# MarkJhonBao/InfantPoseEstimation_GaussianBias

Measured on AMD Instinct MI355X. Metric: images/sec (train fwd+bwd) HRFormer-S 256x192, higher is better.
Workload: dtype bf16; 1 GPU; HRFormer-small + fusion head, 256x192 -> 64x48, K=17, train step fwd+bwd+AdamW, DropPath 0.1, BN train; global_batch=64, per_gpu_batch=64, parallelism=dp1, launch=hipGraph replay, branches on concurrent HIP streams

## Files before the change

include/posekernels.h:

```cpp
#ifndef POSEKERNELS_H
#define POSEKERNELS_H

#include <stdint.h>

#ifdef __cplusplus
extern "C" {
#endif

#define PK_OK 0
#define PK_ERR_INVALID (-1)
#define PK_ERR_UNSUPPORTED (-2)

#define PK_DT_F32 0
#define PK_DT_BF16 1

int pk_version(void);
const char* pk_last_error_string(void);
int pk_marker(int id, void* stream);

int pk_gaussian_target(const float* keypoints, const float* visible, const float* lut, int lut_len,
                       float* target, float* weight, int B, int K, int Hh, int Wh,
                       double stride_x, double stride_y, double reach, int patch_n, int patch_c, void* stream);

int pk_dense_target(const float* keypoints, const float* visible, float* heatmaps, float* weights,
// ... 51 lines not shown
                       int B, int K, int H, int W, float sigma_t, const float* lambdas7, void* stream);

int pk_fusion_terms_fwd(const float* heatmaps, const float* offsets, const float* variances, const float* target,
                        const float* weight, const float* gt_keypoints, const float* coords, float* ws, float* losses, float* sigma,
                        int B, int K, int H, int W, float in_w, float in_h, float sigma_t,
                        const float* lambdas7, int use_target_weight, void* stream);
int pk_fusion_terms_bwd(const float* heatmaps, const float* target, const float* ws, const float* grad_total,
                        const float* grad_sigma, const float* grad_losses ,
                        float* d_heatmaps, float* d_offsets, float* d_variances, float* d_coords,
                        int B, int K, int H, int W, float sigma_t, const float* lambdas7, void* stream);
int pk_local_gaussian_refine(const float* heatmaps, const float* coords_in, float* coords_out, int BK, int H, int W,
                             int local_radius, void* stream);
int pk_softargmax_bwd(const float* heatmaps, const float* coords, const float* scores, const float* grad_coords,
                      const float* grad_scores, float* d_heatmaps, int BK, int H, int W, void* stream);

#define PK_REDUCE_BLOCKS 1024
int pk_pixel_loss_fwd(const float* pred, const float* target, const float* weight, float* partial, float* loss,
                      int B, int K, int HW, int kind, void* stream);
int pk_pixel_loss_bwd(const float* pred, const float* target, const float* weight, const float* grad_out,
                      float* d_pred, int B, int K, int HW, int kind, void* stream);
int pk_spatial_stats(const float* heatmaps, float* mean, float* var, int BK, int H, int W, void* stream);
int pk_spatial_stats_bwd(const float* heatmaps, const float* mean, const float* var, const float* grad_mean, const float* grad_var,
                         float* grad_heatmaps, int BK, int H, int W, void* stream);

int pk_adamw_step(float* param, const float* grad, float* exp_avg, float* exp_avg_sq, const uint8_t* decay_mask,
                  uint16_t* param_bf16, int64_t n, const float* lr_dev, const int32_t* step_dev,
                  float beta1, float beta2, float eps, float weight_decay, float grad_scale, void* stream);



int pk_conv2d_nhwc(const void* x, const void* w_packed, void* out, float* stats_partial, const float* bias,
                   int B, int Hs, int Ws, int Cin, int Cout, int ksize, int stride, int dilated_input, int Ho, int Wo,
                   int act, int out_mode, const void* addend, void* stream);
int pk_conv2d_affine_nhwc(const void* x, const void* w_packed, void* out, const float* col_scale, const float* col_shift,
                          const void* residual, int relu, int B, int Hs, int Ws, int Cin, int Cout, int ksize, int stride, int Ho,
                          int Wo, void* stream);
int pk_conv_stats_tiles(int M);
#define PK_GROUP_MAX 12
typedef struct PkConvDesc {
    const void* x; const void* w; void* out;
    float* stats;
    const float* col_scale;
    const float* bias;
    const void* res;
    int B, Hs, Ws, Cin, Cout, ksize, stride, dilated_input, Ho, Wo;
    int act;
} PkConvDesc;
int pk_conv2d_group(const PkConvDesc* descs, int n, void* stream);
typedef struct PkBnFwdDesc {
    const void* raw; const float* stats_partial; const float* gamma; const float* beta;
    float* running_mean; float* running_var; int64_t* num_batches_tracked;
    const void* residual; void* y; float* save_mean; float* save_rstd; uint8_t* relu_mask ;
    int64_t rows; int tiles, C; float momentum, eps; int relu;
} PkBnFwdDesc;
int pk_bn_train_fwd_group(const PkBnFwdDesc* descs, int n, void* stream);
typedef struct PkBnBwdDesc {
    const void* dy; const void* y_act; const void* raw; const float* save_mean; const float* save_rstd; const float* gamma;
    float* partial; float* dgamma; float* dbeta; void* dx; void* dresidual; const uint8_t* relu_mask ;
    int64_t rows; int C; int relu;
} PkBnBwdDesc;
int pk_bn_bwd_group_blocks(int64_t rows);
int pk_bn_bwd_group(const PkBnBwdDesc* descs, int n, void* stream);
typedef struct PkFuseDesc {
    const void* inputs[4]; int in_h[4]; int in_w[4]; int n_inputs;
    void* out; const void* mask_y; int B, H, W, C, relu;
} PkFuseDesc;
// ... 114 lines not shown
```

infantposeestimation_gaussianbias_amd/csrc/pk_igemm.hip:

```cpp
#include "pk_common.h"

typedef __attribute__((ext_vector_type(8))) short bf16x8;
typedef __attribute__((ext_vector_type(4))) float f32x4;

#define STAT_ROWS 128
#define BKK 32
#define LDS_PITCH 40

struct IgemmArgs {
    const uint16_t* x;
    const uint16_t* w;
    void* out;
    const float* bias;
    const float* col_scale;
    const uint16_t* res;
    const float* res_scale;
    const int32_t* a_rowmap;
    const int32_t* o_rowmap;
    float* stats;
    uint16_t* preact;
    const uint16_t* gelu_of;
    int M, N, Cin, T;
    int Hs, Ws;
    int Ho, Wo;
// ... 562 lines not shown
template <int BM, int BN, int WM, int WN, int BK, int LEAN>
__global__ void __launch_bounds__(256) __attribute__((amdgpu_waves_per_eu(2))) k_igemm2(IgemmArgs p_in) {
    igemm2_body<BM, BN, WM, WN, BK, LEAN>(p_in, (int)blockIdx.x, (int)blockIdx.y, (int)gridDim.x, (int)gridDim.y);
}

struct IgemmGroup {
    IgemmArgs a[PK_GROUP_MAX];
    int first[PK_GROUP_MAX + 1];
    int gy[PK_GROUP_MAX];
    int n;
};
template <int BM, int BN, int WM, int WN, int BK, int LEAN>
__global__ void __launch_bounds__(256) __attribute__((amdgpu_waves_per_eu(2))) k_igemm2g(IgemmGroup g) {
    const int L = (int)blockIdx.x;
    int i = 0;
    while (i + 1 < g.n && L >= g.first[i + 1]) ++i;
    const int local = L - g.first[i], gy = g.gy[i], gx = (g.first[i + 1] - g.first[i]) / gy;
    igemm2_body<BM, BN, WM, WN, BK, LEAN>(g.a[i], local % gx, local / gx, gx, gy);
}

#define C8_STAGE 32768
#define C8_STAGES 5
template <int OFF>
__device__ __forceinline__ bf16x8 c8_read(uint32_t lds_byte_addr) {
    bf16x8 v;
    asm volatile("ds_read_b128 %0, %1 offset:%2" : "=v"(v) : "v"(lds_byte_addr), "n"(OFF) : "memory");
    return v;
}
__device__ __forceinline__ void c8_fence4(bf16x8& a, bf16x8& b, bf16x8& c, bf16x8& d) {
    asm volatile("s_waitcnt lgkmcnt(0)" : "+v"(a), "+v"(b), "+v"(c), "+v"(d)::"memory");
}
__device__ __forceinline__ void c8_barrier() { asm volatile("s_barrier" ::: "memory"); }

__global__ void __launch_bounds__(512, 2) k_conv8p(IgemmArgs p) {
    __shared__ __attribute__((aligned(1024))) uint16_t c8_smem[C8_STAGES * C8_STAGE / 2];
    const int tid = threadIdx.x, lane = tid & 63;
    const int wave = __builtin_amdgcn_readfirstlane(tid >> 6);
    const int grp = wave >> 2;
    const int wn = wave & 3;
    int mt, nt;
    {
        const int G = gridDim.x, L = blockIdx.x, q = G >> 3, r = G & 7, xcd = L & 7;
        const int tile = (xcd < r ? xcd * (q + 1) : r * (q + 1) + (xcd - r) * q) + (L >> 3);
        const int ntiles = p.N >> 8;
        mt = tile / ntiles;
        nt = tile - mt * ntiles;
    }
    const int m0 = mt * 256, n0 = nt * 256;
    const auto rx = __builtin_amdgcn_make_buffer_rsrc(const_cast<uint16_t*>(p.x), 0, 0x7ffffff0, 0x00020000);
    const auto rw = __builtin_amdgcn_make_buffer_rsrc(const_cast<uint16_t*>(p.w), 0, 0x7ffffff0, 0x00020000);
    const uint32_t lds0 = (uint32_t)(uintptr_t)(__attribute__((address_space(3))) void*)c8_smem;

    const int drow = wave * 16 + (lane >> 2);
    const int lchunk = (lane & 3) ^ (((lane >> 5) & 1) << 1);
    unsigned pc[2];
    int pedge[2];
    unsigned wo[2];
    {
        const int hw = p.Ho * p.Wo;
#pragma unroll
        for (int i = 0; i < 2; ++i) {
            const int m = m0 + i * 128 + drow;
            pc[i] = OOB_OFF;
            pedge[i] = 0;
            if (m < p.M) {
                const int b = m / hw, rr = m - b * hw, oy = rr / p.Wo, ox = rr - oy * p.Wo;
                pc[i] = (unsigned)(((b * p.Hs + oy) * p.Ws + ox) * p.Cin + lchunk * 8) * 2u;
                pedge[i] = (oy > 0 ? 1 : 0) | (oy < p.Hs - 1 ? 2 : 0) | (ox > 0 ? 4 : 0) | (ox < p.Ws - 1 ? 8 : 0);
            }
            wo[i] = (unsigned)(((n0 + i * 128 + drow) * p.T) * p.Cin + lchunk * 8) * 2u;
        }
    }
    const int nk = p.T * (p.Cin >> 5);
    int q_tap = 0, q_c0 = 0, q_need = 0, q_delta = 0;
    auto set_tap = [&]() {
        if (p.T == 9) {
            const int kh = q_tap / 3, kw = q_tap - kh * 3;
            q_need = (kh == 0 ? 1 : 0) | (kh == 2 ? 2 : 0) | (kw == 0 ? 4 : 0) | (kw == 2 ? 8 : 0);
            q_delta = ((kh - 1) * p.Ws + (kw - 1)) * p.Cin * 2;
        }
    };
    set_tap();
    auto issue_tile = [&](int stage) {
#if defined(__HIP_DEVICE_COMPILE__)
        uint16_t* sp = c8_smem + (stage * C8_STAGE + wave * 1024) / 2;
#pragma unroll
        for (int i = 0; i < 2; ++i) {
            const bool ok = pc[i] != OOB_OFF && (pedge[i] & q_need) == q_need;
            __builtin_amdgcn_raw_ptr_buffer_load_lds(rx, (__attribute__((address_space(3))) void*)(sp + i * 4096), 16,
                                                     ok ? pc[i] + (unsigned)q_delta : OOB_OFF, q_c0 * 2, 0, 0);
        }
#pragma unroll
        for (int i = 0; i < 2; ++i)
            __builtin_amdgcn_raw_ptr_buffer_load_lds(rw, (__attribute__((address_space(3))) void*)(sp + 8192 + i * 4096), 16, wo[i],
                                                     (q_tap * p.Cin + q_c0) * 2, 0, 0);
#endif
        if (++q_tap == p.T) {
            q_tap = 0;
            q_c0 += 32;
        }
        set_tap();
    };

    const int frow = lane & 15;
    const uint32_t fchunk = (uint32_t)(((lane >> 4) ^ ((frow >> 3) << 1)) * 16);
    const uint32_t faddr_p = lds0 + (grp * 128 + frow) * 64 + fchunk;
    const uint32_t faddr_w = lds0 + 16384 + (wn * 64 + frow) * 64 + fchunk;

    f32x4 acc[4][8];
#pragma unroll
    for (int a = 0; a < 4; ++a)
#pragma unroll
        for (int b = 0; b < 8; ++b) acc[a][b] = (f32x4){0.f, 0.f, 0.f, 0.f};

    issue_tile(0);
    issue_tile(1);
    issue_tile(2);
    asm volatile("s_waitcnt vmcnt(8)" ::: "memory");
    c8_barrier();
    int st_r = 0, st_w = 3;
    bf16x8 wf[4], pf[8];
    auto multiply = [&]() {
        c8_fence4(wf[0], wf[1], wf[2], wf[3]);
        c8_fence4(pf[0], pf[1], pf[2], pf[3]);
        c8_fence4(pf[4], pf[5], pf[6], pf[7]);
        __builtin_amdgcn_sched_barrier(0);
        __builtin_amdgcn_s_setprio(1);
#pragma unroll
        for (int b = 0; b < 8; ++b)
#pragma unroll
            for (int a = 0; a < 4; ++a) acc[a][b] = __builtin_amdgcn_mfma_f32_16x16x32_bf16(wf[a], pf[b], acc[a][b], 0, 0, 0);
        __builtin_amdgcn_s_setprio(0);
// ... 1 lines not shown
    };
    for (int t = 0; t <= nk; ++t) {
        if (grp == 1 && t > 0) multiply();
        if (t < nk) {
            const uint32_t bp = faddr_p + st_r * C8_STAGE, bw = faddr_w + st_r * C8_STAGE;
            wf[0] = c8_read<0>(bw);
            wf[1] = c8_read<1024>(bw);
            wf[2] = c8_read<2048>(bw);
            wf[3] = c8_read<3072>(bw);
            pf[0] = c8_read<0>(bp);
            pf[1] = c8_read<1024>(bp);
            pf[2] = c8_read<2048>(bp);
            pf[3] = c8_read<3072>(bp);
            pf[4] = c8_read<4096>(bp);
            pf[5] = c8_read<5120>(bp);
            pf[6] = c8_read<6144>(bp);
            pf[7] = c8_read<7168>(bp);
            if (t + 3 < nk) issue_tile(st_w);
            __builtin_amdgcn_sched_barrier(0);
            if (grp == 0) multiply();
        }
        if (t + 3 < nk) {
            asm volatile("s_waitcnt vmcnt(8)" ::: "memory");
        } else if (t + 2 < nk) {
            asm volatile("s_waitcnt vmcnt(4)" ::: "memory");
        } else {
            asm volatile("s_waitcnt vmcnt(0)" ::: "memory");
        }
        st_r = st_r == C8_STAGES - 1 ? 0 : st_r + 1;
        st_w = st_w == C8_STAGES - 1 ? 0 : st_w + 1;
        c8_barrier();
    }

    if (p.stats && m0 + grp * 128 < p.M) {
        float* dst = p.stats + (size_t)(mt * 2 + grp) * 2 * p.N + n0 + wn * 64;
#pragma unroll
        for (int a = 0; a < 4; ++a)
#pragma unroll
            for (int r = 0; r < 4; ++r) {
                float sm = 0.f, sq = 0.f;
#pragma unroll
                for (int b = 0; b < 8; ++b) {
                    const float v = acc[a][b][r];
                    sm += v;
                    sq += v * v;
                }
                sm = row16_sum(sm);
                sq = row16_sum(sq);
                if ((lane & 15) == 0) {
                    const int nl = a * 16 + (lane >> 4) * 4 + r;
                    dst[nl] = sm;
                    dst[p.N + nl] = sq;
                }
            }
    }
    uint16_t* stage = c8_smem + wave * 8192;
    if (p.col_scale) {
#pragma unroll
        for (int a = 0; a < 4; ++a) {
            const int c = n0 + wn * 64 + a * 16 + (lane >> 4) * 4;
            const f32x4 sc = *reinterpret_cast<const f32x4*>(p.col_scale + c), sh = *reinterpret_cast<const f32x4*>(p.bias + c);
#pragma unroll
            for (int b = 0; b < 8; ++b) {
                acc[a][b] = acc[a][b] * sc + sh;
                if (p.act == 3) {
#pragma unroll
                    for (int r = 0; r < 4; ++r) acc[a][b][r] = fmaxf(acc[a][b][r], 0.f);
                }
            }
        }
    }
#pragma unroll
    for (int a = 0; a < 4; ++a)
#pragma unroll
        for (int b = 0; b < 8; ++b) {
            const int px = b * 16 + (lane & 15);
            const int chunk = (a * 2 + (lane >> 5)) ^ (px & 7);
            uint2 v;
            v.x = pack_bf16x2(acc[a][b][0], acc[a][b][1]);
            v.y = pack_bf16x2(acc[a][b][2], acc[a][b][3]);
            *reinterpret_cast<uint2*>(stage + px * 64 + chunk * 8 + ((lane >> 4) & 1) * 4) = v;
        }
    __builtin_amdgcn_fence(__ATOMIC_ACQ_REL, "wavefront");
    __builtin_amdgcn_wave_barrier();
    uint16_t* out = reinterpret_cast<uint16_t*>(p.out);
#pragma unroll 4
    for (int it = 0; it < 16; ++it) {
        const int px = it * 8 + (lane >> 3), ch = lane & 7;
        const int m = m0 + grp * 128 + px;
        const u32x4 v = *reinterpret_cast<const u32x4*>(stage + px * 64 + ((ch ^ (px & 7)) * 8));
        if (m < p.M) *reinterpret_cast<u32x4*>(out + (size_t)m * p.ldo + n0 + wn * 64 + ch * 8) = v;
    }
}
typedef __attribute__((ext_vector_type(2))) unsigned int u32x2;
template <int OFF>
__device__ __forceinline__ bf16x8 h3_read(uint32_t lds_byte_addr) {
    bf16x8 v;
    asm volatile("ds_read_b128 %0, %1 offset:%2" : "=v"(v) : "v"(lds_byte_addr), "n"(OFF) : "memory");
    return v;
}
__device__ __forceinline__ int h3_div(int q, int d, float inv) {
    int r = (int)((float)q * inv);
    const int rem = q - r * d;
    r += rem >= d ? 1 : (rem < 0 ? -1 : 0);
    return r;
}
__device__ __forceinline__ void h3_wait_vm(int n) {
#define H3_W(k) case k: asm volatile("s_waitcnt vmcnt(" #k ")" ::: "memory"); break;
    switch (n < 0 ? 0 : (n > 63 ? 63 : n)) {
        H3_W(0) H3_W(1) H3_W(2) H3_W(3) H3_W(4) H3_W(5) H3_W(6) H3_W(7) H3_W(8) H3_W(9) H3_W(10) H3_W(11) H3_W(12) H3_W(13) H3_W(14) H3_W(15)
        H3_W(16) H3_W(17) H3_W(18) H3_W(19) H3_W(20) H3_W(21) H3_W(22) H3_W(23) H3_W(24) H3_W(25) H3_W(26) H3_W(27) H3_W(28) H3_W(29) H3_W(30) H3_W(31)
        H3_W(32) H3_W(33) H3_W(34) H3_W(35) H3_W(36) H3_W(37) H3_W(38) H3_W(39) H3_W(40) H3_W(41) H3_W(42) H3_W(43) H3_W(44) H3_W(45) H3_W(46) H3_W(47)
        H3_W(48) H3_W(49) H3_W(50) H3_W(51) H3_W(52) H3_W(53) H3_W(54) H3_W(55) H3_W(56) H3_W(57) H3_W(58) H3_W(59) H3_W(60) H3_W(61) H3_W(62) H3_W(63)
    }
#undef H3_W
}
template <int CIN, int COUT>
__global__ void __launch_bounds__(256, 2) k_conv3h(IgemmArgs p, int pieces_per_wave) {
    constexpr int RB = CIN * 2, CH = CIN / 8, RP = 1024 / RB, KS = CIN / 32, NI = COUT / 32;
    extern __shared__ __attribute__((aligned(1024))) uint16_t h3_smem[];
    const int tid = threadIdx.x, lane = tid & 63;
    const int wave = __builtin_amdgcn_readfirstlane(tid >> 6);
    const int wm = wave >> 1, wn = wave & 1;
    const int H = p.Hs, W = p.Ws, W2 = W + 2, P = (H + 2) * W2, halo = W + 3;
    const int nsamples = p.M / (H * W), Mp = nsamples * P;
    const int ntiles = (Mp + 127) >> 7;
// ... 317 lines not shown
    }
    PK_REQUIRE((int64_t)M * (ldo > Cin ? ldo : Cin) < 0x3fffffffLL, "%s: tensor too large for 32-bit byte offsets", who);
    return PK_OK;
}

extern "C" int pk_conv2d_nhwc(const void* x, const void* w_packed, void* out, float* stats_partial, const float* bias,
                              int B, int Hs, int Ws, int Cin, int Cout, int ksize, int stride, int dilated_input, int Ho,
                              int Wo, int act, int out_mode, const void* addend, void* stream) {
    const int M = B * Ho * Wo;
    int rc = check_common("pk_conv2d_nhwc", x, w_packed, out, M, Cout, Cin, Cout, out_mode);
    if (rc) return rc;
    PK_REQUIRE(ksize == 1 || ksize == 3, "pk_conv2d_nhwc: ksize %d", ksize);
    PK_REQUIRE(stride == 1 || (stride == 2 && !dilated_input), "pk_conv2d_nhwc: stride %d", stride);
    PK_REQUIRE(B > 0 && Hs > 0 && Ws > 0 && Ho > 0 && Wo > 0, "pk_conv2d_nhwc: bad geometry");
    if (dilated_input) {
        PK_REQUIRE(Ho <= 2 * Hs && Wo <= 2 * Ws && Ho >= 2 * Hs - 1 && Wo >= 2 * Ws - 1, "pk_conv2d_nhwc: dilated geometry %dx%d <- %dx%d", Ho, Wo, Hs, Ws);
    } else {
        const int pad = ksize / 2;
        PK_REQUIRE(Ho == (Hs + 2 * pad - ksize) / stride + 1 && Wo == (Ws + 2 * pad - ksize) / stride + 1,
                   "pk_conv2d_nhwc: output %dx%d does not match input %dx%d k=%d s=%d", Ho, Wo, Hs, Ws, ksize, stride);
    }
    PK_REQUIRE(out_mode >= 0 && out_mode <= 2 && act >= 0 && act <= 2, "pk_conv2d_nhwc: bad mode");
    PK_REQUIRE((int64_t)B * Hs * Ws * Cin < 0x3fffffffLL && (int64_t)Cout * ksize * ksize * Cin < 0x3fffffffLL,
               "pk_conv2d_nhwc: input too large for 32-bit byte offsets");
    PK_REQUIRE(out_mode == 2 || (Cout & 3) == 0, "pk_conv2d_nhwc: Cout=%d must be a multiple of 4 for row-major output", Cout);
    IgemmArgs a{};
    a.x = (const uint16_t*)x; a.w = (const uint16_t*)w_packed; a.out = out; a.bias = bias; a.stats = stats_partial;
    a.M = M; a.N = Cout; a.Cin = Cin; a.T = ksize * ksize; a.Hs = Hs; a.Ws = Ws; a.Ho = Ho; a.Wo = Wo;
    a.stride = stride; a.pad = ksize / 2; a.dilated = dilated_input; a.ldo = Cout; a.rows_per_sample = Ho * Wo;
    a.act = act; a.out_mode = out_mode;
    PK_REQUIRE(!addend || (out_mode == 0 && !stats_partial), "pk_conv2d_nhwc: an addend needs the bf16 row-major output and no statistics");
    a.res = (const uint16_t*)addend;
    return igemm_launch(a, (hipStream_t)stream, "pk_conv2d_nhwc");
}

extern "C" int pk_conv2d_affine_nhwc(const void* x, const void* w_packed, void* out, const float* col_scale, const float* col_shift,
                                     const void* residual, int relu, int B, int Hs, int Ws, int Cin, int Cout, int ksize, int stride, int Ho,
                                     int Wo, void* stream) {
    const int M = B * Ho * Wo;
    int rc = check_common("pk_conv2d_affine_nhwc", x, w_packed, out, M, Cout, Cin, Cout, 0);
    if (rc) return rc;
    PK_REQUIRE(col_scale && col_shift, "pk_conv2d_affine_nhwc: null scale / shift");
    PK_REQUIRE((ksize == 1 || ksize == 3) && (stride == 1 || stride == 2), "pk_conv2d_affine_nhwc: ksize %d stride %d", ksize, stride);
    PK_REQUIRE(B > 0 && Hs > 0 && Ws > 0 && Ho > 0 && Wo > 0, "pk_conv2d_affine_nhwc: bad geometry");
    const int pad = ksize / 2;
    PK_REQUIRE(Ho == (Hs + 2 * pad - ksize) / stride + 1 && Wo == (Ws + 2 * pad - ksize) / stride + 1,
               "pk_conv2d_affine_nhwc: output %dx%d does not match input %dx%d k=%d s=%d", Ho, Wo, Hs, Ws, ksize, stride);
    PK_REQUIRE((int64_t)B * Hs * Ws * Cin < 0x3fffffffLL && (int64_t)Cout * ksize * ksize * Cin < 0x3fffffffLL,
               "pk_conv2d_affine_nhwc: input too large for 32-bit byte offsets");
    PK_REQUIRE((Cout & 3) == 0, "pk_conv2d_affine_nhwc: Cout=%d must be a multiple of 4", Cout);
    IgemmArgs a{};
    a.x = (const uint16_t*)x; a.w = (const uint16_t*)w_packed; a.out = out; a.bias = col_shift; a.col_scale = col_scale;
    a.M = M; a.N = Cout; a.Cin = Cin; a.T = ksize * ksize; a.Hs = Hs; a.Ws = Ws; a.Ho = Ho; a.Wo = Wo;
    a.stride = stride; a.pad = pad; a.dilated = 0; a.ldo = Cout; a.rows_per_sample = Ho * Wo;
    a.act = relu ? 3 : 0; a.out_mode = 0; a.res = (const uint16_t*)residual;
    return igemm_launch(a, (hipStream_t)stream, "pk_conv2d_affine_nhwc");
}

extern "C" int pk_conv2d_group(const PkConvDesc* d, int n, void* stream) {
    PK_REQUIRE(d && n > 0 && n <= PK_GROUP_MAX, "pk_conv2d_group: 1..%d members, got %d", PK_GROUP_MAX, n);
    IgemmGroup g{};
    bool k64 = true;
    int total = 0;
    for (int i = 0; i < n; ++i) {
        const PkConvDesc& c = d[i];
        const int M = c.B * c.Ho * c.Wo;
// ... 1209 lines not shown
```

infantposeestimation_gaussianbias_amd/dispatch.py:

```python
import contextlib
import os

import torch

from . import nnops
from ._lib import PoseKernelError

_ACTIVE = []


def backend_for(model):
    ok = getattr(model, "_pk_supported", None)
    if ok is None:
        ok = nnops.supported(model)
        object.__setattr__(model, "_pk_supported", ok)
    if not ok:
        raise PoseKernelError(
            f"{type(model).__name__}: layer shapes outside the HIP kernels (channels must be multiples of 8, head_dim a multiple of 8 "
            "up to 64, window 7) and no 8-aligned padded twin could be built (models/padded.py); there is no fallback path")
    return nnops


def padded_twin(model):
    if getattr(model, "_pk_twin", None) is False:
        return None
    from .models import padded
    return padded.twin_for(model)


def backend_name(model) -> str:
    if torch.cuda.is_available() and padded_twin(model) is not None:
        return "hip (8-aligned padded twin)"
    backend_for(model)
    return "hip"


@contextlib.contextmanager
def scope(model):
    if _ACTIVE:
        yield _ACTIVE[-1]
        return
    ops = backend_for(model)
    _ACTIVE.append(ops)
    try:
        with nnops.use_weights(model):
            yield ops
            join_detached()
    finally:
        _ACTIVE.pop()


def ops():
    if not _ACTIVE:
        raise RuntimeError("network op called outside dispatch.scope(model)")
    return _ACTIVE[-1]


from .nnops import (backward_milestone, conv_bn_act, deconv_bn_relu, drop_scales, exchange, exchange_output, head_out, mlp_rows, residual_block,
                    to_features, window_attention_tokens, window_block)


def to_public(x):
    ops()
    return x.permute(0, 3, 1, 2)


def from_public(x):
    ops()
    if x.dtype != nnops.ACT_DTYPE:
        B, C, H, W = x.shape
        if x.requires_grad and torch.is_grad_enabled() and C % 8 == 0:
            return x.permute(0, 2, 3, 1).to(nnops.ACT_DTYPE).contiguous()
        return nnops.to_features(x, cpad=-(-C // 8) * 8)
    return x.permute(0, 2, 3, 1).contiguous()


_SIDE = {}
_STREAMS_OFF = [False]
_REGION = [False]
_EVENTS = []


def set_streams(enabled: bool):
    _STREAMS_OFF[0] = not enabled


def set_region_mode(enabled: bool):
    _REGION[0] = bool(enabled)


def streams_enabled() -> bool:
# ... 179 lines not shown
```

infantposeestimation_gaussianbias_amd/models/fusion_head.py:

```python
import math
from typing import Dict, Optional, Tuple

import torch
import torch.nn as nn

from .. import hipops
from .. import dispatch as nnops
from ._blocks import conv


class SoftArgmax2D(nn.Module):

    def __init__(self, beta: float = 1.0):
        super().__init__()
        self.beta = beta

    def forward(self, heatmaps: torch.Tensor) -> Tuple[torch.Tensor, torch.Tensor]:
        h = heatmaps.float()
        if torch.is_grad_enabled() and h.requires_grad:
            co, sc = hipops.softargmax(h)
            if self.beta != 1.0:
                co = hipops.softargmax(h * self.beta)[0]
            return co, sc
        one = torch.full((1,), 40.0, device=heatmaps.device)
# ... 31 lines not shown
    seq = nn.ModuleDict({"0": conv(cin, hidden, 3), "1": nn.BatchNorm2d(hidden), "3": nn.Conv2d(hidden, cout, 1)})
    return seq


class HeatmapRegressionHead(nn.Module):
    def __init__(self, in_channels: int, num_keypoints: int = 17, hidden_dim: int = 256, use_subpixel_refinement: bool = True):
        super().__init__()
        self.in_channels, self.num_keypoints, self.use_subpixel_refinement = in_channels, num_keypoints, use_subpixel_refinement
        self.shared_layers = nn.ModuleDict({"0": conv(in_channels, hidden_dim, 3), "1": nn.BatchNorm2d(hidden_dim),
                                            "3": conv(hidden_dim, hidden_dim, 3), "4": nn.BatchNorm2d(hidden_dim)})
        self.heatmap_branch = _branch(hidden_dim, hidden_dim, num_keypoints)
        self.offset_branch = _branch(hidden_dim, hidden_dim, num_keypoints * 2)
        self.variance_branch = _branch(hidden_dim, hidden_dim // 2, num_keypoints)
        if use_subpixel_refinement:
            self.subpixel_refine = SubPixelRefinement(1.0, 2, 0.5)
        self.fusion_weight = nn.Parameter(torch.tensor(0.5))
        for m in self.modules():
            if isinstance(m, nn.Conv2d):
                nn.init.kaiming_normal_(m.weight, mode="fan_out", nonlinearity="relu")
                if m.bias is not None:
                    nn.init.zeros_(m.bias)

    def forward(self, x: torch.Tensor) -> Dict[str, torch.Tensor]:
        with nnops.scope(self):
            return self._forward(x)

    def _forward(self, x: torch.Tensor) -> Dict[str, torch.Tensor]:
        tr = self.training
        x = nnops.from_public(x)
        s = self.shared_layers
        f = nnops.conv_bn_act(x, s["0"], s["1"], True, None, tr)
        f = nnops.conv_bn_act(f, s["3"], s["4"], True, None, tr)

        def make(br, softplus=False):
            def run(ins):
                t = nnops.conv_bn_act(ins[0], br["0"], br["1"], True, None, tr)
                return nnops.head_out(t, br["3"], softplus)
            return run

        heatmaps, offsets, variances = nnops.parallel([make(self.heatmap_branch), make(self.offset_branch), make(self.variance_branch, True)],
                                                      [[f], [f], [f]])
        B, _, H, W = offsets.shape
        return {"heatmaps": heatmaps, "offsets": offsets.view(B, self.num_keypoints, 2, H, W),
                "variances": variances, "fusion_weight": torch.sigmoid(self.fusion_weight)}

    @torch.no_grad()
    def decode(self, outputs: Dict[str, torch.Tensor], apply_offset: bool = True) -> Tuple[torch.Tensor, torch.Tensor]:
        hm = outputs["heatmaps"].float()
        if self.use_subpixel_refinement:
            alpha, radius = self.subpixel_refine.alpha.detach(), self.subpixel_refine.local_radius
        else:
            alpha, radius = torch.full((1,), 40.0, device=hm.device), 0
        if not apply_offset:
            return hipops.softargmax_refine_decode(hm, None, alpha, None, radius)
        fw = outputs["fusion_weight"].detach().float().reshape(1)
        raw = torch.log(fw / (1 - fw))
        return hipops.softargmax_refine_decode(hm, outputs["offsets"].float(), alpha, raw, radius)


_TERM = {"heatmap": 0, "offset": 1, "peak": 2, "variance": 3, "overlap": 4, "shape": 5}


def _lam(dev, thr=0.5, **terms):
    v = [0.0] * 6 + [float(thr)]
    for k, w in terms.items():
        v[_TERM[k]] = float(w)
    return torch.tensor(v, dtype=torch.float32, device=dev)


class GaussianDistributionConstraint(nn.Module):
    SKELETON = [(0, 1), (0, 2), (1, 3), (2, 4), (5, 6), (5, 7), (7, 9), (6, 8), (8, 10), (5, 11), (6, 12), (11, 12),
                (11, 13), (13, 15), (12, 14), (14, 16)]

# ... 72 lines not shown
```

infantposeestimation_gaussianbias_amd/nnops.py:

```python
import os

import numpy as np
import torch

from . import _lib
from ._lib import call, stream_ptr

BF16, F32, I32 = torch.bfloat16, torch.float32, torch.int32
ACT_DTYPE = BF16
WS = 7


def _e(shape, dtype, dev):
    return torch.empty(shape, dtype=dtype, device=dev)


_SINK_EPOCH = [0]


def begin_grad_epoch():
    _SINK_EPOCH[0] += 1


def sink_written(param) -> bool:
    return getattr(param, "_pk_epoch", -1) == _SINK_EPOCH[0]


def grad_sink_of(param):
    dst = getattr(param, "_pk_grad_sink", None)
    if dst is not None:
        if getattr(param, "_pk_epoch", -1) == _SINK_EPOCH[0] and _SINK_EPOCH[0] > 0:
            raise _lib.PoseKernelError("gradient sink requested twice in one step: a parameter applied more than once per forward (or a "
# ... 269 lines not shown
    layout = 1 if (geom is not None and oihw) else 0
    n_bias = 0 if dbias is None else dbias.numel()
    if deferred and out is not None and deferral_enabled():
        ws = _workspace(out, "w", S * N * (T * Cin + 1))
        call("pk_wgrad_bf16", x, g, ws, None, None, n_bias, a_map, g_map, g_scale, g_rps, M, N, Cin, ksize, stride, B, Hs, Ws, Ho, Wo,
             layout, stream_ptr())
        total = N * T * Cin
        _defer(ws.data_ptr(), out, total, S, total, layout, N, T, Cin)
        if n_bias:
            _defer(ws.data_ptr() + 4 * S * total, dbias, N, S, n_bias)
        return out
    ws = _e((S * N * (T * Cin + 1),), F32, x.device)
    dw = out if out is not None else _e((N, Cin, ksize, ksize) if geom is not None else (N, Cin), F32, x.device)
    call("pk_wgrad_bf16", x, g, ws, dw, dbias, n_bias, a_map, g_map, g_scale, g_rps, M, N, Cin, ksize,
         stride, B, Hs, Ws, Ho, Wo, layout, stream_ptr())
    return dw


def _colsum(g, rows, N, rowmap=None, row_scale=None, rps=0, out=None):
    nb = _lib.lib.pk_ln_bwd_blocks(rows)
    part = _e((nb, N), F32, g.device)
    out = out if out is not None else _e((N,), F32, g.device)
    call("pk_colsum_bf16", g, rowmap, row_scale, rps, part, out, rows, N, stream_ptr())
    return out


class SkipGrad:
    __slots__ = ("g",)

    def __init__(self):
        self.g = None


def _bn_eval_affine(wc, bn, gamma, beta):
    key = (gamma.data_ptr(), gamma._version, beta.data_ptr(), beta._version, bn.running_mean.data_ptr(), bn.running_mean._version,
           bn.running_var.data_ptr(), bn.running_var._version)
    ent = wc.bn_eval.get(id(bn))
    if ent is None or ent[0] != key:
        rstd = torch.rsqrt(bn.running_var + 1e-5)
        scale = gamma * rstd
        shift = torch.addcmul(beta, bn.running_mean, scale, value=-1.0)
        ent = wc.bn_eval[id(bn)] = (key, scale.float().contiguous(), shift.float().contiguous(), bn.running_mean.clone(), rstd)
    return ent[1:]


class _ConvBnAct(torch.autograd.Function):
    @staticmethod
    def forward(ctx, x, weight, gamma, beta, residual, bn, stride, relu, training, skip_out=None, skip_in=None, infer=False):
        ctx.params = (weight, gamma, beta)
        ctx.skip_out, ctx.skip_in = skip_out, skip_in
        wc = _wc()
        wf, wd = wc.fwd[id(weight)], wc.dgrad[id(weight)]
        Cout, Cin_real, ksize = weight.shape[0], weight.shape[1], weight.shape[2]
        x = x.contiguous()
        B, Hs, Ws, Cin, Ho, Wo = _conv_geometry(x, ksize, stride)
        M = B * Ho * Wo
        dev = x.device
        res = None if residual is None else residual.contiguous()
        if infer and not training and os.environ.get("POSE_FUSED_EVAL_BN", "1") != "0":
            scale, shift = _bn_eval_affine(wc, bn, gamma, beta)[:2]
            y = _e((B, Ho, Wo, Cout), BF16, dev)
            call("pk_conv2d_affine_nhwc", x, wf, y, scale, shift, res, 1 if relu else 0, B, Hs, Ws, Cin, Cout, ksize, stride, Ho, Wo, stream_ptr())
            return y
        raw, part = _conv_raw(x, wf, Cout, ksize, stride, training)
        scale, shift = _e((Cout,), F32, dev), _e((Cout,), F32, dev)
        mean, rstd = _e((Cout,), F32, dev), _e((Cout,), F32, dev)
        y = _e(raw.shape, BF16, dev)
        mask = _e((M * Cout // 8,), torch.uint8, dev) if (relu and not infer) else None
        if training:
            wc.bn_eval.pop(id(bn), None)
            call("pk_bn_train_fwd", raw, part, part.shape[0], Cout, M, gamma, beta, bn.running_mean, bn.running_var, bn.num_batches_tracked,
                 0.1, 1e-5, res, y, mean, rstd, scale, shift, 1 if relu else 0, mask, stream_ptr())
        else:
            scale, shift, mean, rstd = _bn_eval_affine(wc, bn, gamma, beta)
            call("pk_bn_act", raw, scale, shift, res, y, M, Cout, 1 if relu else 0, mask, stream_ptr())
        ctx.save_for_backward(x, raw, y if mask is None else mask, mean, rstd, gamma, wd)
        ctx.has_mask = mask is not None
        ctx.meta = (stride, relu, training, residual is not None, Cin_real, ksize, (B, Hs, Ws, Ho, Wo))
        return y

    @staticmethod
    def backward(ctx, dy):
        x, raw, y, mean, rstd, gamma, wd = ctx.saved_tensors
        stride, relu, training, has_res, Cin_real, ksize, (B, Hs, Ws, Ho, Wo) = ctx.meta
        dev, Cout, Cin, M = dy.device, raw.shape[-1], x.shape[-1], B * Ho * Wo
        dy = dy.contiguous()
        nb = _lib.lib.pk_bn_bwd_blocks(M)
        w_p, g_p, b_p = ctx.params
        part, sums = _e((nb, 2, Cout), F32, dev), _e((2 * Cout,), F32, dev)
        (dgamma, sg), (dbeta, sb) = _sink(g_p), _sink(b_p)
        draw = _e(raw.shape, BF16, dev)
        dres = _e(raw.shape, BF16, dev) if has_res else None
        call("pk_bn_bwd", dy, None if ctx.has_mask else y, raw, mean, rstd, gamma, part, sums, dgamma, dbeta, draw, dres, M, Cout,
             (1 if relu else 0) | (0 if training else 2), y if ctx.has_mask else None, stream_ptr())
        addend = None
        if ctx.skip_in is not None:
            addend, ctx.skip_in.g = ctx.skip_in.g, None
            if addend is None:
                raise _lib.PoseKernelError("residual block backward out of order: the skip gradient has not been produced yet")
        if ctx.skip_out is not None:
            ctx.skip_out.g, dres = dres, None
        dx = _conv_dgrad(draw, wd, Cin, ksize, stride, (Hs, Ws), addend) if (ctx.needs_input_grad[0] or addend is not None) else None
        if Cin != Cin_real:
            dw = _wgrad(x, draw, Cout, Cin, ksize, stride, (B, Hs, Ws, Ho, Wo))[:, :Cin_real].contiguous()
            dst = grad_sink_of(w_p)
            if dst is not None:
                dst.copy_(dw)
                dw = None
        else:
            dst, sw = _sink(w_p)
            dw = _wgrad(x, draw, Cout, Cin, ksize, stride, (B, Hs, Ws, Ho, Wo), out=dst, deferred=sw)
            dw = None if sw else dw
        return dx, dw, None if sg else dgamma, None if sb else dbeta, dres, None, None, None, None, None, None, None


def conv_bn_act(x, conv, bn, relu=False, residual=None, training=False, skip_out=None, skip_in=None):
    return _ConvBnAct.apply(x, conv.weight, bn.weight, bn.bias, residual, bn, conv.stride[0], relu, training, skip_out, skip_in,
                            not torch.is_grad_enabled())


def residual_block(x, first, middle, last, training):
    fuse = training and torch.is_grad_enabled() and x.requires_grad and first[0].stride[0] == 1
    hold = SkipGrad() if fuse else None
    y = conv_bn_act(x, first[0], first[1], True, None, training, skip_in=hold)
    for conv, bn in middle:
        y = conv_bn_act(y, conv, bn, True, None, training)
    return conv_bn_act(y, last[0], last[1], True, x.detach() if fuse else x, training, skip_out=hold)


_SHUFFLE_MAPS = {}


def _deconv_taps(k):
    p = (k - 1) // 2
    if k - 2 * p - 2 < 0:
        raise ValueError(f"ConvTranspose2d kernel {k}: output_padding {k - 2 * p - 2} (the reference's rule, pose_estimator.py:53-54) is negative")
    one = []
    for par in (0, 1):
        for kk in range(k):
            if (par + p - kk) % 2 == 0 and -1 <= (par + p - kk) // 2 <= 1:
                one.append((par, (par + p - kk) // 2, kk))
    return [(py * 2 + px, (dy + 1) * 3 + (dx + 1), ky, kx) for py, dy, ky in one for px, dx, kx in one]


class _StackDeconv(torch.autograd.Function):

    @staticmethod
    def forward(ctx, w):
        Cin, Cout, k, _ = w.shape
        ws = torch.zeros(4 * Cout, Cin, 3, 3, dtype=F32, device=w.device)
        for cls, tap, ky, kx in _deconv_taps(k):
# ... 695 lines not shown
```

Measured before the change: 4203 images/sec.

## Merge fusion-head branch data gradients into one multi-source dgrad kernel

The three fusion-head branch convolutions no longer compute their own input gradients in backward. Each hands its BN-backward gradient and dgrad weights to a shared holder, and a new autograd node sums all three data gradients with one implicit-GEMM launch. That launch walks the concatenated K dimension across the sources, which removes two extra kernel launches and the read-modify-write of dx between them. In exchange, the three concurrently running branch backwards must synchronise before the merged kernel, which reduces stream overlap and adds Python-side bookkeeping. When the shapes do not suit the multi kernel, it falls back to chained launches.

```diff
diff --git a/include/posekernels.h b/include/posekernels.h
--- a/include/posekernels.h
+++ b/include/posekernels.h
@@ -107,6 +107,8 @@
 int pk_conv2d_nhwc(const void* x, const void* w_packed, void* out, float* stats_partial, const float* bias,
                    int B, int Hs, int Ws, int Cin, int Cout, int ksize, int stride, int dilated_input, int Ho, int Wo,
                    int act, int out_mode, const void* addend, void* stream);
+int pk_conv2d_dgrad_multi(const void* const* g, const void* const* w_packed, const int* couts, int n_src, void* dx,
+                          const void* addend, int B, int H, int W, int Cin, int ksize, void* stream);
 int pk_conv2d_affine_nhwc(const void* x, const void* w_packed, void* out, const float* col_scale, const float* col_shift,
                           const void* residual, int relu, int B, int Hs, int Ws, int Cin, int Cout, int ksize, int stride, int Ho,
                           int Wo, void* stream);
diff --git a/infantposeestimation_gaussianbias_amd/csrc/pk_igemm.hip b/infantposeestimation_gaussianbias_amd/csrc/pk_igemm.hip
--- a/infantposeestimation_gaussianbias_amd/csrc/pk_igemm.hip
+++ b/infantposeestimation_gaussianbias_amd/csrc/pk_igemm.hip
@@ -618,7 +618,14 @@
 }
 __device__ __forceinline__ void c8_barrier() { asm volatile("s_barrier" ::: "memory"); }
 
-__global__ void __launch_bounds__(512, 2) k_conv8p(IgemmArgs p) {
+struct C8Segs {
+    const uint16_t* x[3];
+    const uint16_t* w[3];
+    int cin[3];
+    int n;
+};
+template <bool MULTI>
+__device__ __forceinline__ void conv8p_body(const IgemmArgs& p, const C8Segs& sg) {
     __shared__ __attribute__((aligned(1024))) uint16_t c8_smem[C8_STAGES * C8_STAGE / 2];
     const int tid = threadIdx.x, lane = tid & 63;
     const int wave = __builtin_amdgcn_readfirstlane(tid >> 6);
@@ -635,6 +642,9 @@
     const int m0 = mt * 256, n0 = nt * 256;
     const auto rx = __builtin_amdgcn_make_buffer_rsrc(const_cast<uint16_t*>(p.x), 0, 0x7ffffff0, 0x00020000);
     const auto rw = __builtin_amdgcn_make_buffer_rsrc(const_cast<uint16_t*>(p.w), 0, 0x7ffffff0, 0x00020000);
+    auto rx_s = rx, rw_s = rw;
+    int cin_s = p.Cin, q_seg = 0;
+#define C8_CIN (MULTI ? cin_s : p.Cin)
     const uint32_t lds0 = (uint32_t)(uintptr_t)(__attribute__((address_space(3))) void*)c8_smem;
 
     const int drow = wave * 16 + (lane >> 2);
@@ -642,6 +652,7 @@
     unsigned pc[2];
     int pedge[2];
     unsigned wo[2];
+    int pix[2];
     {
         const int hw = p.Ho * p.Wo;
 #pragma unroll
@@ -649,21 +660,23 @@
             const int m = m0 + i * 128 + drow;
             pc[i] = OOB_OFF;
             pedge[i] = 0;
+            if (MULTI) pix[i] = -1;
             if (m < p.M) {
                 const int b = m / hw, rr = m - b * hw, oy = rr / p.Wo, ox = rr - oy * p.Wo;
+                if (MULTI) pix[i] = (b * p.Hs + oy) * p.Ws + ox;
                 pc[i] = (unsigned)(((b * p.Hs + oy) * p.Ws + ox) * p.Cin + lchunk * 8) * 2u;
                 pedge[i] = (oy > 0 ? 1 : 0) | (oy < p.Hs - 1 ? 2 : 0) | (ox > 0 ? 4 : 0) | (ox < p.Ws - 1 ? 8 : 0);
             }
             wo[i] = (unsigned)(((n0 + i * 128 + drow) * p.T) * p.Cin + lchunk * 8) * 2u;
         }
     }
-    const int nk = p.T * (p.Cin >> 5);
+    const int nk = p.T * ((MULTI ? sg.cin[0] + sg.cin[1] + (sg.n > 2 ? sg.cin[2] : 0) : p.Cin) >> 5);
     int q_tap = 0, q_c0 = 0, q_need = 0, q_delta = 0;
     auto set_tap = [&]() {
         if (p.T == 9) {
             const int kh = q_tap / 3, kw = q_tap - kh * 3;
             q_need = (kh == 0 ? 1 : 0) | (kh == 2 ? 2 : 0) | (kw == 0 ? 4 : 0) | (kw == 2 ? 8 : 0);
-            q_delta = ((kh - 1) * p.Ws + (kw - 1)) * p.Cin * 2;
+            q_delta = ((kh - 1) * p.Ws + (kw - 1)) * C8_CIN * 2;
         }
     };
     set_tap();
@@ -673,17 +686,29 @@
 #pragma unroll
         for (int i = 0; i < 2; ++i) {
             const bool ok = pc[i] != OOB_OFF && (pedge[i] & q_need) == q_need;
-            __builtin_amdgcn_raw_ptr_buffer_load_lds(rx, (__attribute__((address_space(3))) void*)(sp + i * 4096), 16,
+            __builtin_amdgcn_raw_ptr_buffer_load_lds(MULTI ? rx_s : rx, (__attribute__((address_space(3))) void*)(sp + i * 4096), 16,
                                                      ok ? pc[i] + (unsigned)q_delta : OOB_OFF, q_c0 * 2, 0, 0);
         }
 #pragma unroll
         for (int i = 0; i < 2; ++i)
-            __builtin_amdgcn_raw_ptr_buffer_load_lds(rw, (__attribute__((address_space(3))) void*)(sp + 8192 + i * 4096), 16, wo[i],
-                                                     (q_tap * p.Cin + q_c0) * 2, 0, 0);
+            __builtin_amdgcn_raw_ptr_buffer_load_lds(MULTI ? rw_s : rw, (__attribute__((address_space(3))) void*)(sp + 8192 + i * 4096), 16, wo[i],
+                                                     (q_tap * C8_CIN + q_c0) * 2, 0, 0);
 #endif
         if (++q_tap == p.T) {
             q_tap = 0;
             q_c0 += 32;
+            if (MULTI && q_c0 == cin_s && q_seg + 1 < sg.n) {
+                ++q_seg;
+                q_c0 = 0;
+                cin_s = q_seg == 1 ? sg.cin[1] : sg.cin[2];
+                rx_s = __builtin_amdgcn_make_buffer_rsrc(const_cast<uint16_t*>(q_seg == 1 ? sg.x[1] : sg.x[2]), 0, 0x7ffffff0, 0x00020000);
+                rw_s = __builtin_amdgcn_make_buffer_rsrc(const_cast<uint16_t*>(q_seg == 1 ? sg.w[1] : sg.w[2]), 0, 0x7ffffff0, 0x00020000);
+#pragma unroll
+                for (int i = 0; i < 2; ++i) {
+                    pc[i] = pix[i] < 0 ? OOB_OFF : (unsigned)(pix[i] * cin_s + lchunk * 8) * 2u;
+                    wo[i] = (unsigned)(((n0 + i * 128 + drow) * p.T) * cin_s + lchunk * 8) * 2u;
+                }
+            }
         }
         set_tap();
     };
@@ -751,7 +776,7 @@
         c8_barrier();
     }
 
-    if (p.stats && m0 + grp * 128 < p.M) {
+    if (!MULTI && p.stats && m0 + grp * 128 < p.M) {
         float* dst = p.stats + (size_t)(mt * 2 + grp) * 2 * p.N + n0 + wn * 64;
 #pragma unroll
         for (int a = 0; a < 4; ++a)
@@ -774,7 +799,7 @@
             }
     }
     uint16_t* stage = c8_smem + wave * 8192;
-    if (p.col_scale) {
+    if (!MULTI && p.col_scale) {
 #pragma unroll
         for (int a = 0; a < 4; ++a) {
             const int c = n0 + wn * 64 + a * 16 + (lane >> 4) * 4;
@@ -810,7 +835,10 @@
         const u32x4 v = *reinterpret_cast<const u32x4*>(stage + px * 64 + ((ch ^ (px & 7)) * 8));
         if (m < p.M) *reinterpret_cast<u32x4*>(out + (size_t)m * p.ldo + n0 + wn * 64 + ch * 8) = v;
     }
-}
+#undef C8_CIN
+}
+__global__ void __launch_bounds__(512, 2) k_conv8p(IgemmArgs p) { conv8p_body<false>(p, C8Segs{}); }
+__global__ void __launch_bounds__(512, 2) k_conv8p_multi(IgemmArgs p, C8Segs sg) { conv8p_body<true>(p, sg); }
 typedef __attribute__((ext_vector_type(2))) unsigned int u32x2;
 template <int OFF>
 __device__ __forceinline__ bf16x8 h3_read(uint32_t lds_byte_addr) {
@@ -1194,6 +1222,51 @@
     PK_REQUIRE(!addend || (out_mode == 0 && !stats_partial), "pk_conv2d_nhwc: an addend needs the bf16 row-major output and no statistics");
     a.res = (const uint16_t*)addend;
     return igemm_launch(a, (hipStream_t)stream, "pk_conv2d_nhwc");
+}
+
+extern "C" int pk_conv2d_dgrad_multi(const void* const* g, const void* const* w_packed, const int* couts, int n_src, void* dx,
+                                     const void* addend, int B, int H, int W, int Cin, int ksize, void* stream) {
+    PK_REQUIRE(g && w_packed && couts && dx, "pk_conv2d_dgrad_multi: null pointer");
+    PK_REQUIRE(n_src >= 1 && n_src <= 3, "pk_conv2d_dgrad_multi: 1..3 sources, got %d", n_src);
+    PK_REQUIRE(ksize == 1 || ksize == 3, "pk_conv2d_dgrad_multi: ksize %d", ksize);
+    PK_REQUIRE(B > 0 && H > 0 && W > 0, "pk_conv2d_dgrad_multi: bad geometry");
+    PK_REQUIRE((Cin & 3) == 0, "pk_conv2d_dgrad_multi: Cin=%d must be a multiple of 4", Cin);
+    PK_REQUIRE((((uintptr_t)addend) & 15) == 0, "pk_conv2d_dgrad_multi: addend must be 16-byte aligned");
+    const int M = B * H * W;
+    int total = 0;
+    bool by32 = true;
+    for (int s = 0; s < n_src; ++s) {
+        int rc = check_common("pk_conv2d_dgrad_multi", g[s], w_packed[s], dx, M, Cin, couts[s], Cin, 0);
+        if (rc) return rc;
+        PK_REQUIRE((int64_t)Cin * ksize * ksize * couts[s] < 0x3fffffffLL, "pk_conv2d_dgrad_multi: weight too large for 32-bit byte offsets");
+        total += couts[s];
+        by32 = by32 && (couts[s] % 32) == 0;
+    }
+    IgemmArgs a{};
+    a.out = dx; a.M = M; a.N = Cin; a.T = ksize * ksize; a.Hs = H; a.Ws = W; a.Ho = H; a.Wo = W;
+    a.stride = 1; a.pad = ksize / 2; a.ldo = Cin; a.rows_per_sample = H * W;
+    hipStream_t st = (hipStream_t)stream;
+    if (n_src > 1 && by32 && !addend) {
+        IgemmArgs t = a;
+        t.x = (const uint16_t*)g[0]; t.w = (const uint16_t*)w_packed[0]; t.Cin = total;
+        if (conv8p_takes(t)) {
+            C8Segs sg{};
+            for (int s = 0; s < n_src; ++s) {
+                sg.x[s] = (const uint16_t*)g[s]; sg.w[s] = (const uint16_t*)w_packed[s]; sg.cin[s] = couts[s];
+            }
+            sg.n = n_src;
+            a.x = sg.x[0]; a.w = sg.w[0]; a.Cin = couts[0];
+            hipLaunchKernelGGL(k_conv8p_multi, dim3((unsigned)(((M + 255) / 256) * (Cin / 256))), dim3(512), 0, st, a, sg);
+            return pk_launch_status("pk_conv2d_dgrad_multi");
+        }
+    }
+    for (int s = 0; s < n_src; ++s) {
+        a.x = (const uint16_t*)g[s]; a.w = (const uint16_t*)w_packed[s]; a.Cin = couts[s];
+        a.res = (const uint16_t*)(s == 0 ? addend : dx);
+        int rc = igemm_launch(a, st, "pk_conv2d_dgrad_multi");
+        if (rc) return rc;
+    }
+    return PK_OK;
 }
 
 extern "C" int pk_conv2d_affine_nhwc(const void* x, const void* w_packed, void* out, const float* col_scale, const float* col_shift,
diff --git a/infantposeestimation_gaussianbias_amd/dispatch.py b/infantposeestimation_gaussianbias_amd/dispatch.py
--- a/infantposeestimation_gaussianbias_amd/dispatch.py
+++ b/infantposeestimation_gaussianbias_amd/dispatch.py
@@ -56,7 +56,7 @@
     return _ACTIVE[-1]
 
 
-from .nnops import (backward_milestone, conv_bn_act, deconv_bn_relu, drop_scales, exchange, exchange_output, head_out, mlp_rows, residual_block,
+from .nnops import (backward_milestone, conv_bn_act, deconv_bn_relu, drop_scales, exchange, exchange_output, head_out, merged_dgrad, mlp_rows, residual_block,
                     to_features, window_attention_tokens, window_block)
 
 
diff --git a/infantposeestimation_gaussianbias_amd/models/fusion_head.py b/infantposeestimation_gaussianbias_amd/models/fusion_head.py
--- a/infantposeestimation_gaussianbias_amd/models/fusion_head.py
+++ b/infantposeestimation_gaussianbias_amd/models/fusion_head.py
@@ -87,13 +87,16 @@
         f = nnops.conv_bn_act(x, s["0"], s["1"], True, None, tr)
         f = nnops.conv_bn_act(f, s["3"], s["4"], True, None, tr)
 
-        def make(br, softplus=False):
+        f, hold = nnops.merged_dgrad(f, 3)
+
+        def make(br, softplus=False, dgrad_out=None):
             def run(ins):
-                t = nnops.conv_bn_act(ins[0], br["0"], br["1"], True, None, tr)
+                t = nnops.conv_bn_act(ins[0], br["0"], br["1"], True, None, tr, dgrad_out=dgrad_out)
                 return nnops.head_out(t, br["3"], softplus)
             return run
 
-        heatmaps, offsets, variances = nnops.parallel([make(self.heatmap_branch), make(self.offset_branch), make(self.variance_branch, True)],
+        heatmaps, offsets, variances = nnops.parallel([make(self.heatmap_branch, False, hold[0]), make(self.offset_branch, False, hold[1]),
+                                                       make(self.variance_branch, True, hold[2])],
                                                       [[f], [f], [f]])
         B, _, H, W = offsets.shape
         return {"heatmaps": heatmaps, "offsets": offsets.view(B, self.num_keypoints, 2, H, W),
diff --git a/infantposeestimation_gaussianbias_amd/nnops.py b/infantposeestimation_gaussianbias_amd/nnops.py
--- a/infantposeestimation_gaussianbias_amd/nnops.py
+++ b/infantposeestimation_gaussianbias_amd/nnops.py
@@ -1,3 +1,4 @@
+import ctypes
 import os
 
 import numpy as np
@@ -333,6 +334,58 @@
         self.g = None
 
 
+class DgradHandOver:
+    __slots__ = ("item",)
+
+    def __init__(self):
+        self.item = None
+
+
+def merged_dgrad_enabled() -> bool:
+    return os.environ.get("POSE_MERGED_DGRAD", "1") != "0"
+
+
+class _MergedDgrad(torch.autograd.Function):
+    @staticmethod
+    def forward(ctx, f, holders, ksize):
+        ctx.set_materialize_grads(False)
+        ctx.holders, ctx.ksize, ctx.fshape = holders, ksize, tuple(f.shape)
+        return f.view_as(f)
+
+    @staticmethod
+    def backward(ctx, g):
+        items = []
+        for h in ctx.holders:
+            it, h.item = h.item, None
+            if it is not None:
+                items.append(it)
+        if not items:
+            if g is None:
+                raise _lib.PoseKernelError("merged data gradient: no branch conv has handed over its operands (backward out of order)")
+            return g, None, None
+        B, H, W, C = ctx.fshape
+        cur = torch.cuda.current_stream()
+        for draw, _, _, st in items:
+            if st != cur:
+                if not torch.cuda.is_current_stream_capturing():
+                    cur.wait_stream(st)
+                draw.record_stream(cur)
+        df = _e((B, H, W, C), BF16, items[0][0].device)
+        n = len(items)
+        gp = (ctypes.c_void_p * n)(*[it[0].data_ptr() for it in items])
+        wp = (ctypes.c_void_p * n)(*[it[1].data_ptr() for it in items])
+        cs = (ctypes.c_int * n)(*[it[2] for it in items])
+        call("pk_conv2d_dgrad_multi", gp, wp, cs, n, df, None if g is None else g.contiguous(), B, H, W, C, ctx.ksize, stream_ptr())
+        return df, None, None
+
+
+def merged_dgrad(f, n, ksize=3):
+    if not (torch.is_grad_enabled() and f.requires_grad and merged_dgrad_enabled()):
+        return f, [None] * n
+    holders = [DgradHandOver() for _ in range(n)]
+    return _MergedDgrad.apply(f, holders, ksize), holders
+
+
 def _bn_eval_affine(wc, bn, gamma, beta):
     key = (gamma.data_ptr(), gamma._version, beta.data_ptr(), beta._version, bn.running_mean.data_ptr(), bn.running_mean._version,
            bn.running_var.data_ptr(), bn.running_var._version)
@@ -347,9 +400,12 @@
 
 class _ConvBnAct(torch.autograd.Function):
     @staticmethod
-    def forward(ctx, x, weight, gamma, beta, residual, bn, stride, relu, training, skip_out=None, skip_in=None, infer=False):
+    def forward(ctx, x, weight, gamma, beta, residual, bn, stride, relu, training, skip_out=None, skip_in=None, infer=False, dgrad_out=None):
         ctx.params = (weight, gamma, beta)
         ctx.skip_out, ctx.skip_in = skip_out, skip_in
+        if dgrad_out is not None and (stride != 1 or skip_in is not None or weight.shape[1] != x.shape[-1]):
+            raise _lib.PoseKernelError("conv_bn_act: the data-gradient hand-over needs a stride-1 conv without a skip input")
+        ctx.dgrad_out = dgrad_out
         wc = _wc()
         wf, wd = wc.fwd[id(weight)], wc.dgrad[id(weight)]
         Cout, Cin_real, ksize = weight.shape[0], weight.shape[1], weight.shape[2]
@@ -401,7 +457,13 @@
                 raise _lib.PoseKernelError("residual block backward out of order: the skip gradient has not been produced yet")
         if ctx.skip_out is not None:
             ctx.skip_out.g, dres = dres, None
-        dx = _conv_dgrad(draw, wd, Cin, ksize, stride, (Hs, Ws), addend) if (ctx.needs_input_grad[0] or addend is not None) else None
+        if ctx.dgrad_out is not None:
+            if ctx.dgrad_out.item is not None:
+                raise _lib.PoseKernelError("conv backward ran twice before the merged data gradient consumed its operands")
+            ctx.dgrad_out.item = (draw, wd, Cout, torch.cuda.current_stream())
+            dx = None
+        else:
+            dx = _conv_dgrad(draw, wd, Cin, ksize, stride, (Hs, Ws), addend) if (ctx.needs_input_grad[0] or addend is not None) else None
         if Cin != Cin_real:
             dw = _wgrad(x, draw, Cout, Cin, ksize, stride, (B, Hs, Ws, Ho, Wo))[:, :Cin_real].contiguous()
             dst = grad_sink_of(w_p)
@@ -412,12 +474,12 @@
             dst, sw = _sink(w_p)
             dw = _wgrad(x, draw, Cout, Cin, ksize, stride, (B, Hs, Ws, Ho, Wo), out=dst, deferred=sw)
             dw = None if sw else dw
-        return dx, dw, None if sg else dgamma, None if sb else dbeta, dres, None, None, None, None, None, None, None
-
-
-def conv_bn_act(x, conv, bn, relu=False, residual=None, training=False, skip_out=None, skip_in=None):
+        return dx, dw, None if sg else dgamma, None if sb else dbeta, dres, None, None, None, None, None, None, None, None
+
+
+def conv_bn_act(x, conv, bn, relu=False, residual=None, training=False, skip_out=None, skip_in=None, dgrad_out=None):
     return _ConvBnAct.apply(x, conv.weight, bn.weight, bn.bias, residual, bn, conv.stride[0], relu, training, skip_out, skip_in,
-                            not torch.is_grad_enabled())
+                            not torch.is_grad_enabled(), dgrad_out)
 
 
 def residual_block(x, first, middle, last, training):
```

New measurement: 4233 images/sec, median of 3. Within noise of the previous version (+0.7%).
